# liuli33/CMLPL

Hardware: AMD Instinct MI355X
Metric: HSI patches/sec per training step (higher is better)
Workload: dtype f32 (convolutions: f32 operands as 3 exact bf16 pieces on the bf16 MFMA, 6 of 9 piece products, f32 accumulate, per-product worst case 2^-21 -- conv1's tap loops of the per-sample kernels as 2 fp16 pieces with power-of-two operand scales, 3 piece products, worst case 2^-20 / mean 2^-23, falling back; 1 GPU; B2: synthetic PaviaU-shaped patches 11x11x103, spectrum 103, 9 classes, 128 labelled + 128 unlabelled rows per GPU (batch 256), dual BaseNet2 fwd/bwd + contrastive/mutual losses + bank + Adam, epoch 1 (memory-bank smoothing active), in-kernel PCG4D noise / Philox dropout; global_batch=256, parallelism=dp1

## Files before the change

### cmlpl_amd/csrc/conv3x3.hip

```cpp
#include <stdlib.h>
#include <string.h>
#include <type_traits>

#ifndef CMLPL_ABL
#define CMLPL_ABL 0
#endif
#define CMLPL_UNR_F 1

#include "common.hpp"
#include "kernels.hpp"

namespace cmlpl {

constexpr int CS = 68;

__global__ void pack_weights_kernel(const float* __restrict__ params, long long pstride, PackInfo pi,
                                    float* __restrict__ packed) {
  const int net = blockIdx.y;
  const long long e = (long long)blockIdx.x * blockDim.x + threadIdx.x;
  if (e >= pi.stride) return;
  const float* P = params + (long long)net * pstride;
  float v;
  if (e < 4LL * PACK_B3) {
    const int which = (int)(e / PACK_B3);
// ... 85 lines not shown
#define STAMP(MODE_, i) do {} while (0)
#define STAMPG(MODE_, i) do {} while (0)
#endif

struct Conv3Args {
  const float* in; const uint8_t* mask_in; const float* wpk; const float* bias;
  float* out; uint8_t* mask_out;
  long long in_ns, mask_in_ns, wpk_ns, bias_ns, out_ns, mask_out_ns;
  int n, H, W, S;
  const float* w0t; const float* b0; float* a0out;
  long long w0t_ns, b0_ns;
  int C;
  float* xn_out;
  float* part0; long long part0_ns;
  int bp;
  XSrc xs;
  const float* w2f; long long w2f_ns;
  const float* b2; const float* wc; const float* bc; long long p_ns;
  const float* yin;
  const float* dropmask; float* dropgen; float* catd; float* ynorm; float* logits; float* feat;
  float* p2out; uint8_t* m2out;
  float dropout_p; int train, K;
  const float* dlogits; const float* dfeat; const float* hmask;
  const float* ynrm; const uint8_t* m2in; const float* w2d; long long w2d_ns;
  float* dy; float* dp2out; float* dp1out;
  const float* cube; int crows, ccols; long long pix0; long long* labels_out;
  uint32_t mg_hw, mg_w, mg_p2, mg_w2;
  const float* wpk16; long long wpk16_ns; const uint32_t* h2flag; long long h2flag_ns; int maxslot;
  int h2_noskip;
  int pairshift;
  int hkind;
  uint32_t* hstat;
  const long long* pix;
};

static inline uint32_t fdiv_magic(int d) { return d <= 1 ? 0u : (uint32_t)((0x100000000ULL + (uint32_t)d - 1) / (uint32_t)d); }
__device__ __forceinline__ int fdiv(int x, uint32_t mg) { return mg == 0u ? x : (int)__umulhi((uint32_t)x, mg); }
static inline void conv3_set_magics(Conv3Args& a) {
  const int H2 = a.H >> 1, W2 = a.W >> 1;
  a.mg_hw = fdiv_magic(a.H * a.W); a.mg_w = fdiv_magic(a.W); a.mg_p2 = fdiv_magic(H2 * W2); a.mg_w2 = fdiv_magic(W2);
}

__device__ __forceinline__ void wg_decode(const Conv3Args& a, int& net, int& s0) {
  net = (int)blockIdx.y; s0 = (int)blockIdx.x * a.S;
  if (a.pairshift != 0 && net == 1) { s0 += a.n >> 1; if (s0 >= a.n) s0 -= a.n; }
}
__device__ __forceinline__ int wg_infer_sample(const Conv3Args& a) {
  const int b = (int)blockIdx.x, per = (a.n + 7) >> 3;
  const int s = (b & 7) * per + (b >> 3);
  return ((b >> 3) < per && s < a.n) ? s : -1;
}

typedef float f32x4v __attribute__((ext_vector_type(4)));
__device__ __forceinline__ f32x4v mfma16(float a, float b, f32x4v c) {
  return __builtin_amdgcn_mfma_f32_16x16x4f32(a, b, c, 0, 0, 0);
}

constexpr int SLAB_MAXQ = 16;
constexpr int SLAB_RING = 7;
constexpr int SLAB_WIN = 4;
constexpr int SLAB_NUP = 7;
static_assert(SLAB_NUP == SLAB_RING, "the forward forms the noise of every chunk of a pass up front");
typedef __attribute__((address_space(3))) void slab_lds_void;
typedef __attribute__((address_space(1))) const void slab_gbl_void;
struct SlabRange { const float* xs; int nfl; };
__device__ __forceinline__ SlabRange slab_range(const XSrc& x, int net, int s, int per, int f4base, int nfl) {
// ... 977 lines not shown
    if (sample < a.n) {
      const float* p = c.img + (size_t)(s * c.IMG + (2 * ph + 1) * c.PW + 2 * pw + 1) * CS + c4 * 4;
      const float4 v00 = *(const float4*)p, v01 = *(const float4*)(p + CS);
      const float4 v10 = *(const float4*)(p + c.PW * CS), v11 = *(const float4*)(p + c.PW * CS + CS);
      const size_t g = ((size_t)sample * c.P2 + q) * 64 + c4 * 4;
      float4 o;
      o.x = (v00.x + v01.x + v10.x + v11.x) * 0.25f;
      o.y = (v00.y + v01.y + v10.y + v11.y) * 0.25f;
      o.z = (v00.z + v01.z + v10.z + v11.z) * 0.25f;
      o.w = (v00.w + v01.w + v10.w + v11.w) * 0.25f;
      if constexpr (STORE) *(float4*)(out + g) = o;
      if constexpr (STAT) pmx = mag_max4(pmx, o);
      if (img2 != nullptr) *(float4*)(img2 + (size_t)((ph + 1) * (c.W2 + 2) + pw + 1) * CS + c4 * 4) = o;
#define CMLPL_NIB(A, B, C, D) ((uint32_t)((relu_open(A) ? 1 : 0) | (relu_open(B) ? 2 : 0) | (relu_open(C) ? 4 : 0) | (relu_open(D) ? 8 : 0)))
      const uint32_t m = CMLPL_NIB(v00.x, v01.x, v10.x, v11.x) | (CMLPL_NIB(v00.y, v01.y, v10.y, v11.y) << 8) |
                         (CMLPL_NIB(v00.z, v01.z, v10.z, v11.z) << 16) | (CMLPL_NIB(v00.w, v01.w, v10.w, v11.w) << 24);
#undef CMLPL_NIB
      if constexpr (STORE) *(uint32_t*)(mo + g) = m;
    }
  }
  if constexpr (STAT) { if (statslot != nullptr) h2_publish_max(pmx, statslot); }
}

__device__ __forceinline__ long long logits_argmax(const float* v, int K) {
  int best = 0;
  float bv = v[0];
  for (int k = 1; k < K; ++k) {
    const float x = v[k];
    if (bv == bv && (x != x || x > bv)) { best = k; bv = x; }
  }
  return (long long)best;
}

template <int NW = 4, bool INFER = false>
__device__ __forceinline__ void conv3_fwd_tail(const Conv3Args& a, const Conv3Ctx& c, float* smem) {
  constexpr int NT = 64 * NW;
  const int tid = c.tid, lane = c.lane, wave = c.wave, net = c.net, sample = c.s0;
  const int PW2 = c.W2 + 2;
  const float* img2 = c.wbuf;
  float* row = smem;
  const int SF = 256, F = SF + FD, K = a.K;
  float* red = smem + F;
  const long long rs = (long long)net * a.n + sample;
  constexpr int PS2 = 36;
  const int NPX2 = (c.H2 + 2) * PW2, PLN = NPX2 * PS2;
  uint32_t* pl = (uint32_t*)(smem + 2048);
  auto split_planes = [&]() {
    for (int it = tid; it < NPX2 * 16; it += NT) {
      const int px = it >> 4, c4 = it & 15;
      const float4 v = *(const float4*)(img2 + (size_t)px * CS + 4 * c4);
      const float x[4] = {v.x, v.y, v.z, v.w};
      uint32_t u0[4], u1[4], u2[4];
#pragma unroll
      for (int q = 0; q < 4; ++q) {
        u0[q] = __float_as_uint(x[q]);
        const float r1 = x[q] - __uint_as_float(u0[q] & 0xffff0000u);
        u1[q] = __float_as_uint(r1);
        const float r2 = r1 - __uint_as_float(u1[q] & 0xffff0000u);
        u2[q] = __float_as_uint(r2);
      }
      uint32_t* d = pl + px * PS2 + 2 * c4;
      *(uint2*)(d) = make_uint2(hi_pair(u0[0], u0[1]), hi_pair(u0[2], u0[3]));
      *(uint2*)(d + PLN) = make_uint2(hi_pair(u1[0], u1[1]), hi_pair(u1[2], u1[3]));
      *(uint2*)(d + 2 * PLN) = make_uint2(hi_pair(u2[0], u2[1]), hi_pair(u2[2], u2[3]));
    }
  };
  static_assert(!(INFER && NW == 8), "inference from the cube: four-wave or eight-tile kernels");
  if (NW == 8 && wave >= 4) {
    __syncthreads();
    split_planes();
    __syncthreads();
    __syncthreads();
    __syncthreads();
    __syncthreads();
    return;
  }
  const int j = lane & 15, kg = lane >> 4;
  const uint4* wq = (const uint4*)(a.w2f + (long long)net * a.w2f_ns) + ((kg >> 1) * 6 + (wave >> 1)) * 64 + (kg & 1) * 32 +
                    16 * (wave & 1) + j;
  constexpr int C2_AHEAD = 3;
  uint4 bq[C2_AHEAD + 1][6];
#pragma unroll
  for (int t0 = 0; t0 < C2_AHEAD; ++t0)
#pragma unroll
    for (int ks = 0; ks < 2; ++ks)
#pragma unroll
      for (int pc = 0; pc < 3; ++pc) bq[t0][3 * ks + pc] = wq[((t0 * 4 + 2 * ks) * 3 + pc) * 128];
  const float4 y4 = *(const float4*)(a.yin + rs * FD + 4 * tid);
  const float bias2 = (a.b2 + (long long)net * a.p_ns)[wave * 16 + j];
  const float bcv = (a.bc + (long long)net * a.p_ns)[tid < K ? tid : 0];
  const float* wc = a.wc + (long long)net * a.p_ns;
  const int F4 = F >> 2, fb = wave * F4;
  float wv0[16][5];
#pragma unroll
  for (int q = 0; q < 16; ++q) {
    const float* wr = wc + (long long)(q < K ? q : K - 1) * F + fb + lane;
#pragma unroll
    for (int i = 0; i < 5; ++i) wv0[q][i] = wr[64 * i];
  }
  const int dmode = (!a.train || a.dropout_p <= 0.f) ? 0 : (a.dropmask != nullptr ? 1 : 2);
  const float keep_scale = 1.0f / (1.0f - a.dropout_p);
  float4 dm4[2];
#pragma unroll
  for (int q = 0; q < 2; ++q) {
    const int f0 = 1024 * q + 4 * tid;
    dm4[q] = make_float4(1.f, 1.f, 1.f, 1.f);
    if (f0 < F) {
      if (dmode == 1) {
        dm4[q] = *(const float4*)(a.dropmask + rs * F + f0);
      } else if (dmode == 2) {
        const unsigned long long gs = xsrc_global_sample(a.xs, sample);
        const float4 u = philox_uniform4(a.xs.seed, xsrc_step(a.xs), STREAM_DROPOUT + net, (gs * F + f0) >> 2);
        float4 m4;
        m4.x = (u.x >= a.dropout_p) ? keep_scale : 0.f; m4.y = (u.y >= a.dropout_p) ? keep_scale : 0.f;
        m4.z = (u.z >= a.dropout_p) ? keep_scale : 0.f; m4.w = (u.w >= a.dropout_p) ? keep_scale : 0.f;
        *(float4*)(a.dropgen + rs * F + f0) = m4;
        dm4[q] = m4;
      }
    }
  }
  if (CMLPL_ABL == 25) STAMP(0, 4);
  __syncthreads();
  if (CMLPL_ABL == 25) STAMP(0, 5);
  *(float4*)(row + SF + 4 * tid) = y4;
  split_planes();
  __syncthreads();
  if (CMLPL_ABL == 25) STAMP(0, 6);
  const uint32_t* ap0 = pl + (size_t)(((j >> 2) + 1) * PW2 + (j & 3) + 1) * PS2 + 4 * kg;
  f32x4v acc0 = {0.f, 0.f, 0.f, 0.f}, acc1 = {0.f, 0.f, 0.f, 0.f};
  auto mm = [](const uint4& x, const uint4& y, f32x4v cc) {
    return __builtin_amdgcn_mfma_f32_16x16x32_bf16(__builtin_bit_cast(bf16x8, x), __builtin_bit_cast(bf16x8, y), cc, 0, 0, 0);
  };
  uint4 af[2][6];
  auto read_a = [&](int tap, uint4 (&x)[6]) {
    const uint32_t* ap = ap0 + ((tap / 3 - 1) * PW2 + (tap % 3 - 1)) * PS2;
#pragma unroll
    for (int ks = 0; ks < 2; ++ks) {
      x[3 * ks] = *(const uint4*)(ap + 16 * ks); x[3 * ks + 1] = *(const uint4*)(ap + PLN + 16 * ks);
      x[3 * ks + 2] = *(const uint4*)(ap + 2 * PLN + 16 * ks);
    }
  };
  read_a(0, af[0]);
#pragma unroll
  for (int tap = 0; tap < 9; ++tap) {
    if (tap + C2_AHEAD < 9) {
#pragma unroll
      for (int ks = 0; ks < 2; ++ks)
#pragma unroll
        for (int pc = 0; pc < 3; ++pc)
          bq[(tap + C2_AHEAD) % (C2_AHEAD + 1)][3 * ks + pc] = wq[(((tap + C2_AHEAD) * 4 + 2 * ks) * 3 + pc) * 128];
    }
    if (tap + 1 < 9) read_a(tap + 1, af[(tap + 1) & 1]);
    const uint4 (&bcur)[6] = bq[tap % (C2_AHEAD + 1)];
    const uint4 (&acur)[6] = af[tap & 1];
#pragma unroll
    for (int ks = 0; ks < 2; ++ks) {
      const uint4 a1 = acur[3 * ks], a2 = acur[3 * ks + 1], a3 = acur[3 * ks + 2];
      const uint4 b1 = bcur[3 * ks], b2 = bcur[3 * ks + 1], b3 = bcur[3 * ks + 2];
      acc0 = mm(a1, b3, acc0); acc1 = mm(a2, b2, acc1); acc0 = mm(a3, b1, acc0);
      acc1 = mm(a1, b2, acc1); acc0 = mm(a2, b1, acc0); acc1 = mm(a1, b1, acc1);
    }
    __builtin_amdgcn_sched_group_barrier(0x020, 6, 0);
    __builtin_amdgcn_sched_group_barrier(0x100, 6, 0);
    __builtin_amdgcn_sched_group_barrier(0x008, 12, 0);
  }
  STAMP(0, 8);
  {
    const int co = wave * 16 + j;
    const float* res = img2 + (size_t)((kg + 1) * PW2 + 1) * CS + co;
    float r_[4];
#pragma unroll
    for (int r = 0; r < 4; ++r) r_[r] = relu_nan((acc0[r] + acc1[r]) + bias2 + res[r * CS]);
    const float s0 = r_[0] + r_[1], s1 = r_[2] + r_[3];
    const float t0 = s0 + __shfl_xor(s0, 16, 64), t1 = s1 + __shfl_xor(s1, 16, 64);
    const int dh = kg & 1;
    uint32_t n0 = (relu_open(r_[0]) ? 1u : 0u) | (relu_open(r_[1]) ? 2u : 0u);
    uint32_t n1 = (relu_open(r_[2]) ? 1u : 0u) | (relu_open(r_[3]) ? 2u : 0u);
    n0 <<= 2 * dh; n1 <<= 2 * dh;
    n0 |= (uint32_t)__shfl_xor((int)n0, 16, 64); n1 |= (uint32_t)__shfl_xor((int)n1, 16, 64);
    if (dh == 0) {
      const int ph = kg >> 1;
      const float o0 = t0 * 0.25f, o1 = t1 * 0.25f;
      if constexpr (!INFER) {
        float* p2 = a.p2out + (rs * 4 + ph * 2) * 64 + co;
        uint8_t* m2 = a.m2out + (rs * 4 + ph * 2) * 64 + co;
        p2[0] = o0; p2[64] = o1;
        m2[0] = (uint8_t)n0; m2[64] = (uint8_t)n1;
      }
      row[co * 4 + ph * 2] = o0;
      row[co * 4 + ph * 2 + 1] = o1;
    }
  }
  if (CMLPL_ABL == 25) STAMP(0, 12);
  float ss = (y4.x * y4.x + y4.y * y4.y) + (y4.z * y4.z + y4.w * y4.w);
  ss = wave_sum(ss);
  if (lane == 0) red[wave] = ss;
  __syncthreads();
  if (CMLPL_ABL == 25) STAMP(0, 13);
  if constexpr (!INFER) {
// ... 51 lines not shown
    }
    float t[16];
#pragma unroll
    for (int q = 0; q < 16; ++q) {
      float acc = 0.f;
#pragma unroll
      for (int i = 0; i < 5; ++i) acc = fmaf(xr[i], wv[q][i], acc);
      t[q] = acc;
    }
#pragma unroll
    for (int o = 32; o > 0; o >>= 1)
#pragma unroll
      for (int q = 0; q < 16; ++q) t[q] += __shfl_xor(t[q], o, 64);
    if (lane == 0) {
#pragma unroll
      for (int q = 0; q < 16; ++q)
        if (kc + q < K) part[wave * 64 + kc + q] = t[q];
    }
  }
  __syncthreads();
  if constexpr (INFER) {
    if (tid < K) {
      const float lg = ((part[tid] + part[64 + tid]) + (part[128 + tid] + part[192 + tid])) + bcv;
      part[256 + tid] = lg;
      if (a.logits != nullptr) a.logits[rs * K + tid] = lg;
    }
    __syncthreads();
    if (tid == 0) a.labels_out[rs] = logits_argmax(part + 256, K);
  } else {
    if (tid < K) a.logits[rs * K + tid] = ((part[tid] + part[64 + tid]) + (part[128 + tid] + part[192 + tid])) + bcv;
  }
}

template <int NW = 4>
__device__ __forceinline__ const float* conv3_bwd_head(const Conv3Args& a, float* smem, uint32_t (&mpre)[2]) {
  constexpr int NT = 64 * NW;
  const int tid = threadIdx.x, lane = tid & 63;
  const int wave = __builtin_amdgcn_readfirstlane(tid >> 6);
  int net, sample;
  wg_decode(a, net, sample);
  const int H2 = a.H >> 1, W2 = a.W >> 1, P2 = H2 * W2, PW2 = W2 + 2;
  const int SF = 256, F = SF + FD, K = a.K;
  float* img2 = smem + (size_t)(a.H + 2) * (a.W + 2) * CS;
  float* ext = img2 + WBUF + 128;
  float* dp1s = ext;
  float* dp2s = dp1s + P2 * 64;
  float* dls = dp2s + 256;
  float* red = dls + 64;
  const long long rs = (long long)net * a.n + sample;
#pragma unroll
  for (int q = 0; q < 2; ++q) {
    const int idx = tid + NT * q;
    mpre[q] = (idx < P2 * 16) ? *(const uint32_t*)(a.mask_in + (long long)net * a.mask_in_ns + ((size_t)sample * P2 + (idx >> 4)) * 64 + (idx & 15) * 4) : 0u;
  }
  if (NW == 8 && wave >= 4) {
    __syncthreads(); __syncthreads(); __syncthreads(); __syncthreads(); __syncthreads(); __syncthreads();
    return dp1s;
  }
  const int l31 = lane & 31, hh = lane >> 5;
  const int nt = wave & 1, kh2 = wave >> 1;
  const uint4* wq = (const uint4*)(a.w2d + (long long)net * a.w2d_ns) + lane;
  constexpr int C2_AHEAD = 3;
  uint4 bq[C2_AHEAD + 1][6];
#pragma unroll
  for (int t0 = 0; t0 < C2_AHEAD; ++t0)
#pragma unroll
    for (int q = 0; q < 2; ++q)
#pragma unroll
      for (int pc = 0; pc < 3; ++pc) bq[t0][3 * q + pc] = wq[(size_t)t0 * TAPW + (((kh2 * 2 + q) * 3 + pc) * 2 + nt) * 64];
  if (tid < 64) dls[tid] = (tid < K) ? a.dlogits[rs * K + tid] : 0.f;
  const float* y = a.yin + rs * FD;
  const float* df = (a.dfeat != nullptr) ? a.dfeat + rs * FD : nullptr;
  const float norm = a.ynrm[rs];
  float yv[4], dv[4];
#pragma unroll
  for (int q = 0; q < 4; ++q) {
    yv[q] = y[tid + 256 * q];
    dv[q] = (df != nullptr) ? df[tid + 256 * q] : 0.f;
  }
  const uint32_t m2pre = (tid < 64) ? *(const uint32_t*)(a.m2in + (rs * 4 + (tid >> 4)) * 64 + (tid & 15) * 4) : 0u;
  const float* wc = a.wc + (long long)net * a.p_ns;
  const float* dm = (a.hmask != nullptr) ? a.hmask + rs * F : nullptr;
  float dmv[5];
#pragma unroll
  for (int it = 0; it < 5; ++it) dmv[it] = (dm != nullptr) ? dm[tid + 256 * it] : 1.f;
  float wv0[16][5];
#pragma unroll
  for (int q = 0; q < 16; ++q) {
    const float* wr = wc + (long long)(q < K ? q : K - 1) * F + tid;
#pragma unroll
    for (int it = 0; it < 5; ++it) wv0[q][it] = wr[256 * it];
  }
  {
    const float4 z4 = make_float4(0.f, 0.f, 0.f, 0.f);
    for (int i = tid; i < 1024; i += 256) ((float4*)img2)[i] = z4;
    const int PW = a.W + 2, IMG = (a.H + 2) * PW;
    for (int i = tid; i < IMG * (CS / 4); i += 256) ((float4*)smem)[i] = z4;
    int* lut = (int*)(img2 + WBUF);
    const int HWl = a.H * a.W;
    for (int m = tid; m < 128; m += 256) {
      const int mm = (m < HWl) ? m : 0;
      const int r = mm / a.W, cc = mm - r * a.W;
// ... 54 lines not shown
    const float4 d = *(const float4*)(dp2s + pp * 64 + c4 * 4);
    const uint32_t m = m2pre;
    uint32_t zmx = 0u;
#pragma unroll
    for (int sub = 0; sub < 4; ++sub) {
      float4 v;
      v.x = ((m >> sub) & 1u) ? d.x * 0.25f : 0.f;
      v.y = ((m >> (8 + sub)) & 1u) ? d.y * 0.25f : 0.f;
      v.z = ((m >> (16 + sub)) & 1u) ? d.z * 0.25f : 0.f;
      v.w = ((m >> (24 + sub)) & 1u) ? d.w * 0.25f : 0.f;
      const int h = 2 * ph + (sub >> 1), w = 2 * pw + (sub & 1);
      *(float4*)(img2 + (size_t)((h + 1) * PW2 + w + 1) * CS + c4 * 4) = v;
      zmx = mag_max4(zmx, v);
    }
    if (a.hstat != nullptr) {
      zmx = wave_mag_max(zmx);
      if (tid == 0) { a.hstat[(3 * 2 + net) * a.n + sample] = zmx; ((uint32_t*)smem)[a.maxslot + 1] = zmx; }
    }
  }
  __syncthreads();
  const bool z2skip = a.hstat != nullptr && a.h2_noskip == 0 && ((const volatile uint32_t*)smem)[a.maxslot + 1] == 0u &&
                      a.h2flag[(long long)net * a.h2flag_ns] == 0u;
  STAMP(1, 5);
  const int mg2 = (65536 + W2 - 1) / W2;
  const int phA = (l31 * mg2) >> 16;
  const int posA = l31 < P2 ? (phA + 1) * PW2 + (l31 - phA * W2) + 1 : 0;
  const float* ap = img2 + (size_t)posA * CS + kh2 * 32 + hh * 8;
  f32x16 acc = zero16();
  auto raw_ptr = [&](int u) {
    const int tap = u >> 1;
    const int toff = ((tap / 3 - 1) * PW2 + (tap % 3 - 1)) * CS;
    return ((l31 < P2) ? ap + toff : ap) + 16 * (u & 1);
  };
  ASplit cur;
  float4 rn0, rn1;
  if (!z2skip) {
  {
    const float* p0 = raw_ptr(0);
    a_split(*(const float4*)p0, *(const float4*)(p0 + 4), cur.p1, cur.p2, cur.p3);
    const float* p1 = raw_ptr(1);
    rn0 = *(const float4*)p1; rn1 = *(const float4*)(p1 + 4);
  }
#pragma unroll
  for (int u = 0; u < 18; ++u) {
    const int tap = u >> 1, q = u & 1;
    if (q == 0 && tap + C2_AHEAD < 9) {
#pragma unroll
      for (int q2 = 0; q2 < 2; ++q2)
#pragma unroll
        for (int pc = 0; pc < 3; ++pc)
          bq[(tap + C2_AHEAD) % (C2_AHEAD + 1)][3 * q2 + pc] =
              wq[(size_t)(tap + C2_AHEAD) * TAPW + (((kh2 * 2 + q2) * 3 + pc) * 2 + nt) * 64];
    }
    if (q == 0) __builtin_amdgcn_sched_barrier(0);
    float4 rnn0 = rn0, rnn1 = rn1;
    if (u + 2 < 18) {
      const float* p2 = raw_ptr(u + 2);
      rnn0 = *(const float4*)p2; rnn1 = *(const float4*)(p2 + 4);
    }
    const uint4 (&bcur)[6] = bq[tap % (C2_AHEAD + 1)];
    acc = mfma_b3(cur.p1, cur.p2, cur.p3, bcur[3 * q], bcur[3 * q + 1], bcur[3 * q + 2], acc);
    ASplit nxt = cur;
    if (u + 1 < 18) a_split(rn0, rn1, nxt.p1, nxt.p2, nxt.p3);
    if (u + 2 < 18) __builtin_amdgcn_sched_group_barrier(0x100, 2, 0);
    SchedInterleave<6>::run();
    cur = nxt; rn0 = rnn0; rn1 = rnn1;
  }
  }
  STAMP(1, 6);
// ... 437 lines not shown
        if (p < P2) {
          const float v = (acc[r] + xch[r * 64 + lane]) + res[r];
          dp1s[p * 64 + ci] = v;
          dp1g[p * 64 + ci] = v;
        }
      }
    }
  }
  __syncthreads();
  STAMP(1, 11);
  return dp1s;
}

template <int MODE, int MTW, int TAIL = 0, int NW = 4, int TPW = 8 / NW, bool KSG = false, bool H2X = false>
__global__ __launch_bounds__(64 * NW, ((MODE >= 2 || KSG) && NW == 4 ? 2 : 1)) void conv3x3_kernel(Conv3Args a) {
  static_assert(!KSG || (MODE < 2 && MTW == 1 && TAIL == 0 && NW == 4 && TPW == 2), "KSG: four waves, S = 1, four tiles");
  static_assert(!H2X || (MODE >= 2 && TAIL == 1 && (NW == 8 || TPW == 2)) || (MODE < 2 && TAIL == 0 && (KSG || NW == 8)),
                "H2X: the per-sample kernels with tail / head; the general kernels with one sample per workgroup");
  extern __shared__ __attribute__((aligned(16))) float smem[];
  if constexpr (H2X) { if (threadIdx.x == 0) { smem[a.maxslot] = 0.f; smem[a.maxslot + 1] = 0.f; } }
  constexpr int NT = 64 * NW;
  constexpr int KMT = NW * TPW / 2;
  constexpr int LUTN = (MODE >= 2) ? KMT * 32 : MTW * NW * 32;
  constexpr bool BIG = (KMT == 8);
  constexpr bool INFER = (MODE == 2 && TAIL >= 2);
  if constexpr (INFER) { if (wg_infer_sample(a) < 0) return; }
  if (CMLPL_ABL == 26) return;
  Conv3Ctx c;
  STAMPG(MODE & 1, 0);
  const float* dp_lds = nullptr;
  uint32_t mpre[2] = {0u, 0u};
  if constexpr (MODE == 3 && TAIL) {
    if constexpr (BIG) dp_lds = conv3_bwd_head_g(a, smem, mpre);
    else dp_lds = conv3_bwd_head<NW>(a, smem, mpre);
  }
  conv3_stage<MODE, NW, TPW, INFER ? (TAIL & 1) + 1 : 0, H2X, (INFER && TAIL >= 4)>(a, smem, LUTN, c, dp_lds, mpre);
  STAMPG(MODE & 1, 1);
  const int tid = c.tid, lane = c.lane, l31 = c.l31, hh = c.hh, wave = c.wave, net = c.net, s0 = c.s0;
  const int HW = c.HW, PW = c.PW, S = c.S, PX = c.PX, npx = c.npx;
  float* img = c.img; float* wbuf = c.wbuf; int* lut = c.lut; const float4* wg = c.wg;
  const TapRegs wp = c.wp;
  const int MT = (npx + 31) >> 5;
  int abase[MTW];
  f32x16 acc[MTW][2];
  constexpr bool KS = (MODE >= 2) || KSG;
  const int RL = MT - NW * (MTW - 1);
  const bool nsplit = !KS && NW == 8 && MTW >= 2 && (RL == 1 || RL == 5);
  int last_tile = wave + NW * (MTW - 1), nmask = 3;
  if (nsplit && wave == RL - 1) nmask = 1;
  else if (nsplit && wave == RL) { last_tile = MT - 1; nmask = 2; }
  auto slot_tile = [&](int t) { return t == MTW - 1 ? last_tile : wave + NW * t; };
  if constexpr (!KS) {
#pragma unroll
    for (int t = 0; t < MTW; ++t) {
      abase[t] = lut[slot_tile(t) * 32 + l31] * CS + 8 * hh;
      acc[t][0] = zero16();
      acc[t][1] = zero16();
    }
  }
  int ab2[TPW];
  f32x16 acc2[TPW][2];
  if (KS) {
#pragma unroll
    for (int t = 0; t < TPW; ++t) {
      ab2[t] = lut[(TPW * (wave >> 1) + t) * 32 + l31] * CS + 8 * hh;
      acc2[t][0] = zero16();
      acc2[t][1] = zero16();
// ... 118 lines not shown
      const int nm = (t == MTW - 1) ? nmask : 3;
      if (tile < MT) {
        int pos[16];
        float x0[16], x1[16];
#pragma unroll
        for (int r = 0; r < 16; ++r) {
          const int m = tile * 32 + acc_row(r, lane);
          pos[r] = lut[m < npx ? m : 0] * CS;
        }
#pragma unroll
        for (int r = 0; r < 16; ++r) { x0[r] = img[pos[r] + l31]; x1[r] = img[pos[r] + 32 + l31]; }
#pragma unroll
        for (int r = 0; r < 16; ++r) {
          const int m = tile * 32 + acc_row(r, lane);
          if (m < npx) {
            if (nm & 1) img[pos[r] + l31] = relu_nan(acc[t][0][r] + bv0 + x0[r]);
            if (nm & 2) img[pos[r] + 32 + l31] = relu_nan(acc[t][1][r] + bv1 + x1[r]);
          }
        }
      }
    }
    }
    if (TAIL) {
      const float4 z4 = make_float4(0.f, 0.f, 0.f, 0.f);
      for (int i = tid; i < (BIG ? WBUF / 4 : 1024); i += NT) ((float4*)wbuf)[i] = z4;
    }
    STAMP(0, 10);
    __syncthreads();
    STAMP(0, 11);
    conv3_pool_store<NT, !INFER, H2X>(a, c, TAIL ? wbuf : nullptr, (H2X && a.hstat != nullptr) ? smem + a.maxslot + 1 : nullptr);
    STAMP(0, 7);
    if constexpr (TAIL != 0) {
      if constexpr (BIG) conv3_fwd_tail_g<INFER>(a, c, smem);
      else conv3_fwd_tail<NW, INFER>(a, c, smem);
    }
    if constexpr (H2X) {
      if (a.hstat != nullptr && tid == 0) a.hstat[(1 * 2 + net) * a.n + s0] = ((const volatile uint32_t*)smem)[a.maxslot + 1];
    }
  } else if (MODE == 3) {
    const int C = a.C, BP = a.bp;
    float vv[TPW][16];
    {
      int pos[16];
#pragma unroll
      for (int r = 0; r < 16; ++r) {
        const int m = ot * 32 + acc_row(r, lane);
        pos[r] = lut[m < PX ? m : 0] * CS + 32 * nt0 + l31;
      }
#pragma unroll
      for (int r = 0; r < 16; ++r)
#pragma unroll
        for (int i = 0; i < TPW; ++i) vv[i][r] = img[pos[r] + 32 * i];
#pragma unroll
      for (int r = 0; r < 16; ++r)
#pragma unroll
        for (int i = 0; i < TPW; ++i) vv[i][r] += own[i][r];
    }
    __syncthreads();
    float* slab = smem;
    float* dal = smem + (C < BP ? C : BP) * HW;
    const int Cw = conv0_partial_rows(C);
    float* pp = a.part0 + (long long)net * a.part0_ns + (size_t)s0 * ((size_t)Cw * 64 + 64);
    bool zskip = false;
    if constexpr (H2X) {
      if (a.hstat != nullptr) zskip = hzero && a.h2_noskip == 0 && (a.hstat[(0 * 2 + net) * a.n + s0] >> 23) < 255u;
    }
    SlabRange rg = slab_range(a.xs, net, s0, C * HW, 0, (C < BP ? C : BP) * HW);
// ... 439 lines not shown
  *v = Conv3Variant{};
  if (H != W || K < 1 || K > 64 || C < 1) return false;
  BigGeom g;
  if (conv3_big_geom(H, W, &g) && conv3_big_fwd_lds(g, C) <= LDS_MAX) {
    *v = per_sample(8, 2, conv3_big_fwd_lds(g, C));
    return true;
  }
  if (switches().fuse_conv0 == 0 || switches().fuse_tail == 0 || H * W > 128 || H < 8 || W < 8) return false;
  if (H2 / 2 != 2 || W2 / 2 != 2 || (H2 + 2) * (W2 + 2) * CS > 4096 || !conv3_divide_exact(W, 128)) return false;
  const size_t lds = conv3_fused_lds(H, W, C, conv3_lds(1, H, W, 1));
  if (2 * lds > LDS_MAX) return false;
  *v = per_sample(4, 2, lds);
  return true;
}

static Conv3Args conv3_args(int mode, int n, int H, int W, int S, const float* in, const uint8_t* mask_in, float* out,
                            uint8_t* mask_out) {
  Conv3Args a{};
  const long long window = (long long)n * H * W * 64, pooled = (long long)n * (H / 2) * (W / 2) * 64;
  a.in = in; a.mask_in = mask_in; a.out = out; a.mask_out = mask_out;
  if (in) a.in_ns = mode == 0 ? window : pooled;
  if (mask_in) a.mask_in_ns = pooled;
  if (out) a.out_ns = mode == 1 ? window : pooled;
  if (mask_out) a.mask_out_ns = pooled;
  a.n = n; a.H = H; a.W = W; a.S = S;
  conv3_set_magics(a);
  a.h2_noskip = switches().f16x2 == 4 || switches().zero_skip == 0;
  return a;
}
static void conv3_args_h2x(Conv3Args& a, const Conv3Variant& v, const float* wpk16, long long wpk16_ns, const uint32_t* h2flag,
                           uint32_t* hstat) {
  a.wpk16 = wpk16; a.wpk16_ns = wpk16_ns; a.h2flag = h2flag; a.h2flag_ns = wpk16_ns; a.hstat = hstat; a.maxslot = v.maxslot;
}

template <int MODE, int MTW, int TAIL, int NW, int TPW, bool KSG, bool H2X>
static hipError_t launch_conv3_k(const Conv3Args& a, dim3 grid, size_t lds, hipStream_t st) {
  static DevOnce attr_once;
  if (lds > LDS_MAX) return hipErrorInvalidValue;
  hipError_t e = ensure_max_lds(attr_once, conv3x3_kernel<MODE, MTW, TAIL, NW, TPW, KSG, H2X>);
  if (e != hipSuccess) return e;
  hipLaunchKernelGGL((conv3x3_kernel<MODE, MTW, TAIL, NW, TPW, KSG, H2X>), grid, dim3(64 * NW), lds, st, a);
  return hipGetLastError();
}
template <int MODE>
static hipError_t launch_conv3_small(const Conv3Args& a, dim3 grid, size_t lds, hipStream_t st) {
  static DevOnce attr_once;
  hipError_t e = ensure_max_lds(attr_once, conv3x3_small_kernel<MODE>);
  if (e != hipSuccess) return e;
  hipLaunchKernelGGL((conv3x3_small_kernel<MODE>), grid, dim3(256), lds, st, a);
  return hipGetLastError();
}

struct Conv3Kernel {
  int mode, mtw, tail, nw, tpw; bool ks, h2x;
  hipError_t (*launch)(const Conv3Args&, dim3, size_t, hipStream_t);
};
#define CMLPL_K(...) {__VA_ARGS__, launch_conv3_k<__VA_ARGS__>}
static const Conv3Kernel conv3_kernels[] = {
    CMLPL_K(0, 1, 0, 4, 2, true, true),
    CMLPL_K(1, 1, 0, 4, 2, true, true),
    CMLPL_K(0, 1, 0, 8, 1, false, true),
    CMLPL_K(1, 1, 0, 8, 1, false, true),
    CMLPL_K(0, 2, 0, 8, 1, false, true),
    CMLPL_K(1, 2, 0, 8, 1, false, true),
    CMLPL_K(0, 1, 0, 4, 2, true, false),
    CMLPL_K(1, 1, 0, 4, 2, true, false),
// ... 42 lines not shown
      return k.launch(a, grid, v.lds, st);
  return hipErrorInvalidValue;
}

hipError_t launch_conv3(const Conv3Variant& v, int mode, int nets, int n, int H, int W, const float* in, const uint8_t* mask_in,
                        const float* wpk, long long wpk_ns, const float* bias, long long bias_ns,
                        float* out, uint8_t* mask_out, hipStream_t st, const Conv3H2& h2) {
  if (v.S < 1) return hipErrorInvalidValue;
  Conv3Args a = conv3_args(mode, n, H, W, v.S, in, mask_in, out, mask_out);
  a.wpk = wpk; a.wpk_ns = wpk_ns; a.bias = bias; a.bias_ns = bias_ns;
  if (v.h2x) { conv3_args_h2x(a, v, h2.wpk16, h2.wpk16_ns, h2.h2flag, h2.hstat); a.hkind = h2.kind; }
  const dim3 grid((n + v.S - 1) / v.S, nets);
  return launch_conv3_variant(mode, 0, v, a, grid, st);
}

hipError_t launch_conv3_fused(const NetRoute& r, int nets, int n, int C, int H, int W, const XSrc& xs, const float* w0t,
                              long long w0t_ns, const float* b0, long long b0_ns, float* a0out, const float* wpk,
                              long long wpk_ns, const float* bias, long long bias_ns, float* out, uint8_t* mask_out,
                              const FwdTail* tail, hipStream_t st, float* xn_out) {
  const Conv3Variant& v = r.fwd_ps;
  if (r.fwd != (tail != nullptr ? ROUTE_A : ROUTE_B)) return hipErrorInvalidValue;
  Conv3Args a = conv3_args(2, n, H, W, 1, nullptr, nullptr, out, mask_out);
  a.wpk = wpk; a.wpk_ns = wpk_ns; a.bias = bias; a.bias_ns = bias_ns;
  a.w0t = w0t; a.w0t_ns = w0t_ns; a.b0 = b0; a.b0_ns = b0_ns; a.a0out = a0out; a.C = C; a.xn_out = xn_out;
  a.xs = xs;
  if (tail == nullptr) return launch_conv3_variant(2, 0, v, a, dim3(n, nets), st);
  a.w2f = tail->w2f; a.w2f_ns = tail->w2f_ns; a.b2 = tail->b2; a.wc = tail->wc; a.bc = tail->bc; a.p_ns = tail->p_ns;
  a.yin = tail->y; a.dropmask = tail->dropmask; a.dropgen = tail->dropgen; a.catd = tail->catd; a.ynorm = tail->ynorm;
  a.logits = tail->logits; a.feat = tail->feat; a.p2out = tail->p2; a.m2out = tail->m2;
  a.dropout_p = tail->dropout_p; a.train = tail->train; a.K = tail->K;
  if (v.h2x) {
    if (tail->w1h == nullptr || tail->h2flag == nullptr) return hipErrorInvalidValue;
    conv3_args_h2x(a, v, tail->w1h, tail->w1h_ns, tail->h2flag, tail->hstat);
  }
  return launch_conv3_variant(2, 1, v, a, dim3(n, nets), st);
}

hipError_t launch_conv3_infer(const Conv3Variant& v, int n, int C, int H, int W, const float* cube, int crows, int ccols,
                              long long pix0, const float* w0t, const float* b0, const float* wpk, const float* bias,
                              const FwdTail& t, long long* labels_out, hipStream_t st, const InferNets* nn, const ViewKey* view) {
  const int nets = nn != nullptr ? nn->nets : 1;
  if (v.S != 1 || n < 1 || !cube || !labels_out || nets < 1 || nets > 2) return hipErrorInvalidValue;
  if ((long long)crows * ccols * C >= (1LL << 31) || W / 2 > crows || W / 2 > ccols) return hipErrorInvalidValue;
  Conv3Args a = conv3_args(2, n, H, W, 1, nullptr, nullptr, nullptr, nullptr);
  a.wpk = wpk; a.bias = bias;
  a.w0t = w0t; a.b0 = b0; a.C = C;
  a.w2f = t.w2f; a.b2 = t.b2; a.wc = t.wc; a.bc = t.bc; a.yin = t.y; a.logits = t.logits; a.K = t.K;
  a.cube = cube; a.crows = crows; a.ccols = ccols; a.pix0 = pix0; a.labels_out = labels_out;
  if (nn != nullptr) {
    a.wpk_ns = nn->packed_ns; a.w0t_ns = nn->packed_ns; a.w2f_ns = nn->packed_ns;
    a.bias_ns = nn->param_ns; a.b0_ns = nn->param_ns; a.p_ns = nn->param_ns;
    a.pix = nn->pix;
  }
  const dim3 grid(8 * ((n + 7) / 8), nets);
  if (view != nullptr && view->sigma != 0.f) {
    a.xs.sigma = view->sigma; a.xs.seed = view->seed; a.xs.step = view->view;
    return launch_conv3_variant(2, a.pix != nullptr ? 5 : 4, v, a, grid, st);
  }
  return launch_conv3_variant(2, a.pix != nullptr ? 3 : 2, v, a, grid, st);
}

hipError_t launch_conv3_fused_bwd(const NetRoute& r, int nets, int n, int C, int H, int W, const float* dpool,
                                  const uint8_t* mask, const float* wpk, long long wpk_ns, const XSrc& xs, float* part0,
                                  long long part0_ns, const BwdHead* head, hipStream_t st) {
  const Conv3Variant& v = r.bwd_ps;
  if (r.bwd != (head != nullptr ? ROUTE_A : ROUTE_B)) return hipErrorInvalidValue;
  if (xs.sigma != 0.f || xs.sel.lab_idx != nullptr || xs.sel.unl_idx != nullptr) return hipErrorInvalidValue;
  Conv3Args a = conv3_args(3, n, H, W, 1, dpool, mask, nullptr, nullptr);
  a.wpk = wpk; a.wpk_ns = wpk_ns;
  a.C = C; a.xs = xs; a.part0 = part0; a.part0_ns = part0_ns; a.bp = v.bp;
  if (head == nullptr) return launch_conv3_variant(3, 0, v, a, dim3(n, nets), st);
  a.dlogits = head->dlogits; a.dfeat = head->dfeat; a.hmask = head->mask; a.wc = head->wc; a.p_ns = head->p_ns;
  a.yin = head->y; a.ynrm = head->ynorm; a.m2in = head->m2; a.w2d = head->w2d; a.w2d_ns = head->w2d_ns;
  a.dy = head->dy; a.dp2out = head->dp2; a.dp1out = head->dp1; a.K = head->K;
  a.pairshift = (nets == 2 && switches().bwd_pair != 0) ? 1 : 0;
  if (v.h2x) {
    if (head->w1h == nullptr || head->h2flag == nullptr) return hipErrorInvalidValue;
    conv3_args_h2x(a, v, head->w1h, head->w1h_ns, head->h2flag, head->hstat);
  }
  return launch_conv3_variant(3, 1, v, a, dim3(n, nets), st);
}

}
```

### cmlpl_amd/csrc/kernels.hpp

```cpp
#pragma once
#include <hip/hip_runtime.h>
#include <stdint.h>
#include <stddef.h>
#include <stdlib.h>
#include <atomic>

#include "common.hpp"

namespace cmlpl {

constexpr int PACK_CONV = 9 * 64 * 64;
constexpr int PACK_B3 = PACK_CONV * 3 / 2;
constexpr int PACK_PER_NET = 4 * PACK_B3 + PACK_CONV;
__host__ __device__ inline long long pack_off_b3(int , int , int which) { return (long long)which * PACK_B3; }
__host__ __device__ inline long long pack_off_frag() { return 4LL * PACK_B3; }
__host__ __device__ inline int conv_b3_index(int tap, int k, int n, int p) {
  return ((((tap * 4 + (k >> 4)) * 3 + p) * 2 + (n >> 5)) * 64 + ((k >> 3) & 1) * 32 + (n & 31)) * 8 + (k & 7);
}
__host__ __device__ inline long long pack_off_w0t() { return PACK_PER_NET; }
__host__ __device__ inline long long pack_off_wst(int C) { return PACK_PER_NET + (long long)((C + 1) & ~1) * 64; }
__host__ __device__ inline long long pack_off_w0b3(int C, int bands) { return pack_off_wst(C) + (long long)bands * 1024; }
__host__ __device__ inline long long pack_off_w0b3_end(int C, int bands) { return pack_off_w0b3(C, bands) + (long long)((C + 15) / 16) * 1536; }
constexpr int H2_WEXP = 13;
constexpr int PACK_H2 = PACK_CONV;
// ... 133 lines not shown
hipError_t launch_feat_norm(int nets, int n, const float* y, float* ynorm, float* feat, long long feat_ns, hipStream_t st);
struct GemmTN {
  const float* A; const float* B; float* C; float* bias;
  const float* bias_in; long long bias_in_bstride; int relu;
  long long a_bstride, b_bstride, c_bstride, bias_bstride;
  int lda, ldb, ldc, M, N, R, batches;
  float scale;
  int b_seg_rows = 0; long long b_seg_stride = 0;
};
hipError_t launch_gemm_tn(const GemmTN& g, hipStream_t st);
hipError_t launch_gemm_tn2(const GemmTN& g0, const GemmTN& g1, hipStream_t st);

hipError_t launch_head_fwd(int nets, int n, int HW4, int K, const float* p2, const float* y, const float* dropmask,
                           float* dropgen, float dropout_p, int train, uint64_t seed, uint64_t step,
                           int nlab, int lab0, int unl_base,
                           const float* wc, const float* bc, long long pstride,
                           float* catd, float* ynorm, float* logits, float* feat, hipStream_t st,
                           DynRef dyn = DynRef());
hipError_t launch_head_bwd(int nets, int n, int HW4, int K, const float* dlogits, const float* dfeat,
                           const float* dropmask, const float* wc, long long pstride,
                           const float* y, const float* ynorm,
                           float* dy, float* dp2, hipStream_t st);
hipError_t launch_dy_fixup(int nets, int n, const float* y, const float* ynorm, const float* dfeat, float* dy,
                           hipStream_t st);

struct Switches {
  int fuse_conv0, fuse_conv0_bwd, fuse_tail, fuse_spe;
  int fuse_big;
  int conv3_nw8;
  int conv0a;
  int zero_skip;
  int bwd_pair;
  int f16x2;
  int conv3_ks;
  int ks8;
  int conv3_s, conv0_dma, conv0_ps;
  int wgrad3_u, wgrad3_cspl, wgrad3_r, wgrad3_ru, wgrad3_rg, wgrad3_pg1, wgrad3_pg2, wgrad3_b3, wgrad3_pair;
  int pair_wide, pair_nbw, pair_mb, pair16, pair_tall;
  int dfeat_lds;
  int mb_fast, unsup_onewg, unsup_3l, ntx_mfma;
  int ntx_ncw;
};
inline Switches read_switches() {
    auto env = [](const char* name, int dflt) { const char* v = getenv(name); return v ? atoi(v) : dflt; };
    Switches w;
    w.fuse_conv0 = env("CMLPL_FUSE_CONV0", 1); w.fuse_conv0_bwd = env("CMLPL_FUSE_CONV0_BWD", 1);
    w.fuse_tail = env("CMLPL_FUSE_TAIL", 1); w.fuse_spe = env("CMLPL_FUSE_SPE", 1);
    w.ks8 = env("CMLPL_KS8", -1); w.fuse_big = env("CMLPL_FUSE_BIG", 1); w.conv3_nw8 = env("CMLPL_CONV3_NW8", 1); w.conv3_ks = env("CMLPL_CONV3_KS", 1); w.conv0a = env("CMLPL_CONV0A", 1); w.f16x2 = env("CMLPL_F16X2", 1); w.bwd_pair = env("CMLPL_BWD_PAIR", 1); w.zero_skip = env("CMLPL_ZERO_SKIP", 1);
    w.conv3_s = env("CMLPL_CONV3_S", 0); w.conv0_dma = env("CMLPL_CONV0_DMA", 1); w.conv0_ps = env("CMLPL_CONV0_PS", 0);
    w.wgrad3_u = env("CMLPL_WGRAD3_U", 0); w.wgrad3_cspl = env("CMLPL_WGRAD3_CSPL", 0); w.wgrad3_r = env("CMLPL_WGRAD3_R", 1);
    w.wgrad3_ru = env("CMLPL_WGRAD3_RU", 0); w.wgrad3_rg = env("CMLPL_WGRAD3_RG", 0);
    w.wgrad3_pg1 = env("CMLPL_WGRAD3_PG1", 0); w.wgrad3_pg2 = env("CMLPL_WGRAD3_PG2", 0);
    w.wgrad3_b3 = env("CMLPL_WGRAD3_B3", 1); w.wgrad3_pair = env("CMLPL_WGRAD3_PAIR", 1);
    w.pair_wide = env("CMLPL_PAIR_WIDE", -1); w.pair_nbw = env("CMLPL_PAIR_NBW", 0); w.pair_mb = env("CMLPL_PAIR_MB", 0);
    w.pair16 = env("CMLPL_PAIR16", 1); w.pair_tall = env("CMLPL_PAIR_TALL", -1);
    w.dfeat_lds = env("CMLPL_DFEAT_LDS", -1);
    w.mb_fast = env("CMLPL_MB_FAST", 1); w.unsup_onewg = env("CMLPL_UNSUP_ONEWG", 1); w.unsup_3l = env("CMLPL_UNSUP_3L", 1);
    w.ntx_mfma = env("CMLPL_NTX_MFMA", 1); w.ntx_ncw = env("CMLPL_NTX_NCW", 0);
    return w;
}
inline Switches& switches_table() {
  static Switches sw = read_switches();
  return sw;
}
inline const Switches& switches() { return switches_table(); }

inline int device_cus() {
  static std::atomic<int> cache[64];
  int dev = 0;
  if (hipGetDevice(&dev) != hipSuccess) return 256;
  int v = cache[dev & 63].load(std::memory_order_relaxed);
  if (v == 0) {
    hipDeviceProp_t prop;
    v = (hipGetDeviceProperties(&prop, dev) == hipSuccess && prop.multiProcessorCount > 0) ? prop.multiProcessorCount : 256;
    cache[dev & 63].store(v, std::memory_order_relaxed);
  }
  return v;
}

struct LossArgs {
  const float* logits; const float* feat; const int64_t* labels;
// ... 97 lines not shown
```

Baseline: 1.761 million patches/s.

## Run conv2 fwd tail and bwd head on fp16 two-piece MFMA path

```diff
diff --git a/cmlpl_amd/csrc/conv3x3.hip b/cmlpl_amd/csrc/conv3x3.hip
--- a/cmlpl_amd/csrc/conv3x3.hip
+++ b/cmlpl_amd/csrc/conv3x3.hip
@@ -141,6 +141,7 @@
   int hkind;
   uint32_t* hstat;
   const long long* pix;
+  int h2c2;
 };
 
 static inline uint32_t fdiv_magic(int d) { return d <= 1 ? 0u : (uint32_t)((0x100000000ULL + (uint32_t)d - 1) / (uint32_t)d); }
@@ -1184,7 +1185,7 @@
   return (long long)best;
 }
 
-template <int NW = 4, bool INFER = false>
+template <int NW = 4, bool INFER = false, bool H2X = false>
 __device__ __forceinline__ void conv3_fwd_tail(const Conv3Args& a, const Conv3Ctx& c, float* smem) {
   constexpr int NT = 64 * NW;
   const int tid = c.tid, lane = c.lane, wave = c.wave, net = c.net, sample = c.s0;
@@ -1217,10 +1218,38 @@
       *(uint2*)(d + 2 * PLN) = make_uint2(hi_pair(u2[0], u2[1]), hi_pair(u2[2], u2[3]));
     }
   };
+  bool spec = false, c2h = false;
+  float c2sc = 1.f, c2inv = 1.f;
+  if constexpr (H2X) spec = a.h2c2 != 0 && a.hstat != nullptr && a.h2flag[(long long)net * a.h2flag_ns] == 0u;
+  auto split_planes_h = [&](float sc) {
+    for (int it = tid; it < NPX2 * 16; it += NT) {
+      const int px = it >> 4, c4 = it & 15;
+      const float4 v = *(const float4*)(img2 + (size_t)px * CS + 4 * c4);
+      const float x0 = v.x * sc, x1 = v.y * sc, x2 = v.z * sc, x3 = v.w * sc;
+      const f16x2v p0 = __builtin_bit_cast(f16x2v, __builtin_amdgcn_cvt_pkrtz(x0, x1));
+      const f16x2v p1 = __builtin_bit_cast(f16x2v, __builtin_amdgcn_cvt_pkrtz(x2, x3));
+      uint32_t* d = pl + px * PS2 + 2 * c4;
+      *(uint2*)(d) = make_uint2(__builtin_bit_cast(uint32_t, p0), __builtin_bit_cast(uint32_t, p1));
+      *(uint2*)(d + PLN) = make_uint2(__builtin_bit_cast(uint32_t, __builtin_amdgcn_cvt_pkrtz(x0 - (float)p0[0], x1 - (float)p0[1])),
+                                      __builtin_bit_cast(uint32_t, __builtin_amdgcn_cvt_pkrtz(x2 - (float)p1[0], x3 - (float)p1[1])));
+    }
+  };
+  auto c2_decide = [&]() {
+    if constexpr (H2X) {
+      if (spec) {
+        const uint32_t mxb = __builtin_amdgcn_readfirstlane(((const volatile uint32_t*)smem)[a.maxslot + 1]);
+        const uint32_t e = mxb >> 23;
+        c2h = (e >= 40u && e <= 200u) || mxb == 0u;
+        c2sc = mxb == 0u ? 1.f : __uint_as_float((268u - e) << 23);
+        c2inv = mxb == 0u ? 1.f : __uint_as_float((e - 27u - (uint32_t)(H2_WEXP - 13)) << 23);
+      }
+    }
+  };
   static_assert(!(INFER && NW == 8), "inference from the cube: four-wave or eight-tile kernels");
   if (NW == 8 && wave >= 4) {
     __syncthreads();
-    split_planes();
+    c2_decide();
+    if (c2h) split_planes_h(c2sc); else split_planes();
     __syncthreads();
     __syncthreads();
     __syncthreads();
@@ -1232,24 +1261,42 @@
                     16 * (wave & 1) + j;
   constexpr int C2_AHEAD = 3;
   uint4 bq[C2_AHEAD + 1][6];
-#pragma unroll
-  for (int t0 = 0; t0 < C2_AHEAD; ++t0)
-#pragma unroll
-    for (int ks = 0; ks < 2; ++ks)
-#pragma unroll
-      for (int pc = 0; pc < 3; ++pc) bq[t0][3 * ks + pc] = wq[((t0 * 4 + 2 * ks) * 3 + pc) * 128];
+  auto b3_fill = [&]() {
+#pragma unroll
+    for (int t0 = 0; t0 < C2_AHEAD; ++t0)
+#pragma unroll
+      for (int ks = 0; ks < 2; ++ks)
+#pragma unroll
+        for (int pc = 0; pc < 3; ++pc) bq[t0][3 * ks + pc] = wq[((t0 * 4 + 2 * ks) * 3 + pc) * 128];
+  };
+  const uint4* wqh = nullptr;
+  constexpr int H_AHEAD = C2_AHEAD;
+  auto hq = [&](int tap, int i) -> uint4& { return bq[tap % (H_AHEAD + 1)][i]; };
+  if constexpr (H2X) {
+    wqh = (const uint4*)(a.wpk16 + (long long)net * a.wpk16_ns + 2LL * PACK_H2) + ((kg >> 1) * 4 + (wave >> 1)) * 64 +
+          (kg & 1) * 32 + 16 * (wave & 1) + j;
+    if (spec) {
+#pragma unroll
+      for (int t0 = 0; t0 < H_AHEAD; ++t0)
+#pragma unroll
+        for (int i = 0; i < 4; ++i) hq(t0, i) = wqh[(t0 * 8 + 4 * (i >> 1) + (i & 1)) * 128];
+    }
+  }
+  if (!spec) b3_fill();
   const float4 y4 = *(const float4*)(a.yin + rs * FD + 4 * tid);
   const float bias2 = (a.b2 + (long long)net * a.p_ns)[wave * 16 + j];
   const float bcv = (a.bc + (long long)net * a.p_ns)[tid < K ? tid : 0];
   const float* wc = a.wc + (long long)net * a.p_ns;
   const int F4 = F >> 2, fb = wave * F4;
+  constexpr int WV_EARLY = H2X ? 4 : 16;
   float wv0[16][5];
-#pragma unroll
-  for (int q = 0; q < 16; ++q) {
+  auto wv_load = [&](int q) {
     const float* wr = wc + (long long)(q < K ? q : K - 1) * F + fb + lane;
 #pragma unroll
     for (int i = 0; i < 5; ++i) wv0[q][i] = wr[64 * i];
-  }
+  };
+#pragma unroll
+  for (int q = 0; q < WV_EARLY; ++q) wv_load(q);
   const int dmode = (!a.train || a.dropout_p <= 0.f) ? 0 : (a.dropmask != nullptr ? 1 : 2);
   const float keep_scale = 1.0f / (1.0f - a.dropout_p);
   float4 dm4[2];
@@ -1275,7 +1322,9 @@
   __syncthreads();
   if (CMLPL_ABL == 25) STAMP(0, 5);
   *(float4*)(row + SF + 4 * tid) = y4;
-  split_planes();
+  c2_decide();
+  if (c2h) split_planes_h(c2sc); else split_planes();
+  if (spec && !c2h) b3_fill();
   __syncthreads();
   if (CMLPL_ABL == 25) STAMP(0, 6);
   const uint32_t* ap0 = pl + (size_t)(((j >> 2) + 1) * PW2 + (j & 3) + 1) * PS2 + 4 * kg;
@@ -1292,6 +1341,35 @@
       x[3 * ks + 2] = *(const uint4*)(ap + 2 * PLN + 16 * ks);
     }
   };
+  if (c2h) {
+    auto mh = [](const uint4& x, const uint4& y, f32x4v cc) {
+      return __builtin_amdgcn_mfma_f32_16x16x32_f16(__builtin_bit_cast(f16x8v, x), __builtin_bit_cast(f16x8v, y), cc, 0, 0, 0);
+    };
+    uint4 ah[2][4];
+    auto read_h = [&](int tap, uint4 (&x)[4]) {
+      const uint32_t* ap = ap0 + ((tap / 3 - 1) * PW2 + (tap % 3 - 1)) * PS2;
+#pragma unroll
+      for (int ks = 0; ks < 2; ++ks) { x[2 * ks] = *(const uint4*)(ap + 16 * ks); x[2 * ks + 1] = *(const uint4*)(ap + PLN + 16 * ks); }
+    };
+    read_h(0, ah[0]);
+#pragma unroll
+    for (int tap = 0; tap < 9; ++tap) {
+      const uint4 g[4] = {hq(tap, 0), hq(tap, 1), hq(tap, 2), hq(tap, 3)};
+      if (tap + H_AHEAD < 9) {
+#pragma unroll
+        for (int i = 0; i < 4; ++i) hq(tap + H_AHEAD, i) = wqh[((tap + H_AHEAD) * 8 + 4 * (i >> 1) + (i & 1)) * 128];
+      }
+      if (tap + 1 < 9) read_h(tap + 1, ah[(tap + 1) & 1]);
+      const uint4 (&h)[4] = ah[tap & 1];
+      acc0 = mh(h[1], g[0], acc0); acc1 = mh(h[0], g[1], acc1); acc0 = mh(h[0], g[0], acc0);
+      acc1 = mh(h[3], g[2], acc1); acc0 = mh(h[2], g[3], acc0); acc1 = mh(h[2], g[2], acc1);
+      __builtin_amdgcn_sched_group_barrier(0x020, 4, 0);
+      __builtin_amdgcn_sched_group_barrier(0x100, 4, 0);
+      __builtin_amdgcn_sched_group_barrier(0x008, 6, 0);
+    }
+#pragma unroll
+    for (int r = 0; r < 4; ++r) { acc0[r] = (acc0[r] + acc1[r]) * c2inv; acc1[r] = 0.f; }
+  } else {
   read_a(0, af[0]);
 #pragma unroll
   for (int tap = 0; tap < 9; ++tap) {
@@ -1316,7 +1394,10 @@
     __builtin_amdgcn_sched_group_barrier(0x100, 6, 0);
     __builtin_amdgcn_sched_group_barrier(0x008, 12, 0);
   }
+  }
   STAMP(0, 8);
+#pragma unroll
+  for (int q = WV_EARLY; q < 16; ++q) wv_load(q);
   {
     const int co = wave * 16 + j;
     const float* res = img2 + (size_t)((kg + 1) * PW2 + 1) * CS + co;
@@ -1434,7 +1515,7 @@
   }
 }
 
-template <int NW = 4>
+template <int NW = 4, bool H2X = false>
 __device__ __forceinline__ const float* conv3_bwd_head(const Conv3Args& a, float* smem, uint32_t (&mpre)[2]) {
   constexpr int NT = 64 * NW;
   const int tid = threadIdx.x, lane = tid & 63;
@@ -1464,12 +1545,29 @@
   const uint4* wq = (const uint4*)(a.w2d + (long long)net * a.w2d_ns) + lane;
   constexpr int C2_AHEAD = 3;
   uint4 bq[C2_AHEAD + 1][6];
+  auto b3_fill = [&]() {
 #pragma unroll
   for (int t0 = 0; t0 < C2_AHEAD; ++t0)
 #pragma unroll
     for (int q = 0; q < 2; ++q)
 #pragma unroll
       for (int pc = 0; pc < 3; ++pc) bq[t0][3 * q + pc] = wq[(size_t)t0 * TAPW + (((kh2 * 2 + q) * 3 + pc) * 2 + nt) * 64];
+  };
+  bool spec = false;
+  const uint4* wqh = nullptr;
+  constexpr int H_AHEAD = 5;
+  auto hq = [&](int tap, int i) -> uint4& { const int sl = (tap % (H_AHEAD + 1)) * 4 + i; return bq[sl / 6][sl % 6]; };
+  if constexpr (H2X) {
+    spec = a.h2c2 != 0 && a.hstat != nullptr && a.h2flag[(long long)net * a.h2flag_ns] == 0u;
+    wqh = (const uint4*)(a.wpk16 + (long long)net * a.wpk16_ns + 2LL * PACK_H2) + lane;
+    if (spec) {
+#pragma unroll
+      for (int t0 = 0; t0 < H_AHEAD; ++t0)
+#pragma unroll
+        for (int i = 0; i < 4; ++i) hq(t0, i) = wqh[(size_t)t0 * TAPH + (((kh2 * 2 + (i >> 1)) * 2 + (i & 1)) * 2 + nt) * 64];
+    }
+  }
+  if (!spec) b3_fill();
   if (tid < 64) dls[tid] = (tid < K) ? a.dlogits[rs * K + tid] : 0.f;
   const float* y = a.yin + rs * FD;
   const float* df = (a.dfeat != nullptr) ? a.dfeat + rs * FD : nullptr;
@@ -1590,9 +1688,53 @@
     const int toff = ((tap / 3 - 1) * PW2 + (tap % 3 - 1)) * CS;
     return ((l31 < P2) ? ap + toff : ap) + 16 * (u & 1);
   };
+  bool c2h = false;
+  float c2sc = 1.f, c2inv = 1.f;
+  if constexpr (H2X) {
+    if (spec) {
+      const uint32_t mxb = __builtin_amdgcn_readfirstlane(((const volatile uint32_t*)smem)[a.maxslot + 1]);
+      const uint32_t e = mxb >> 23;
+      c2h = (e >= 40u && e <= 200u) || mxb == 0u;
+      c2sc = mxb == 0u ? 1.f : __uint_as_float((268u - e) << 23);
+      c2inv = mxb == 0u ? 1.f : __uint_as_float((e - 27u - (uint32_t)(H2_WEXP - 13)) << 23);
+    }
+  }
+  if (!z2skip && c2h) {
+    HSplit hc;
+    float4 rn0, rn1;
+    {
+      const float* p0 = raw_ptr(0);
+      h_split(*(const float4*)p0, *(const float4*)(p0 + 4), c2sc, hc.p1, hc.p2);
+      const float* p1 = raw_ptr(1);
+      rn0 = *(const float4*)p1; rn1 = *(const float4*)(p1 + 4);
+    }
+#pragma unroll
+    for (int u = 0; u < 18; ++u) {
+      const int tap = u >> 1, q = u & 1;
+      if (q == 0 && tap + H_AHEAD < 9) {
+#pragma unroll
+        for (int i = 0; i < 4; ++i)
+          hq(tap + H_AHEAD, i) = wqh[(size_t)(tap + H_AHEAD) * TAPH + (((kh2 * 2 + (i >> 1)) * 2 + (i & 1)) * 2 + nt) * 64];
+      }
+      if (q == 0) __builtin_amdgcn_sched_barrier(0);
+      float4 rnn0 = rn0, rnn1 = rn1;
+      if (u + 2 < 18) {
+        const float* p2 = raw_ptr(u + 2);
+        rnn0 = *(const float4*)p2; rnn1 = *(const float4*)(p2 + 4);
+      }
+      acc = mfma_h2(hc.p1, hc.p2, hq(tap, 2 * q), hq(tap, 2 * q + 1), acc);
+      HSplit nxt = hc;
+      if (u + 1 < 18) h_split(rn0, rn1, c2sc, nxt.p1, nxt.p2);
+      if (u + 2 < 18) __builtin_amdgcn_sched_group_barrier(0x100, 2, 0);
+      SchedInterleave<3>::run();
+      hc = nxt; rn0 = rnn0; rn1 = rnn1;
+    }
+#pragma unroll
+    for (int r = 0; r < 16; ++r) acc[r] *= c2inv;
+  } else if (!z2skip) {
   ASplit cur;
   float4 rn0, rn1;
-  if (!z2skip) {
+  if (spec) b3_fill();
   {
     const float* p0 = raw_ptr(0);
     a_split(*(const float4*)p0, *(const float4*)(p0 + 4), cur.p1, cur.p2, cur.p3);
@@ -2096,7 +2238,7 @@
   uint32_t mpre[2] = {0u, 0u};
   if constexpr (MODE == 3 && TAIL) {
     if constexpr (BIG) dp_lds = conv3_bwd_head_g(a, smem, mpre);
-    else dp_lds = conv3_bwd_head<NW>(a, smem, mpre);
+    else dp_lds = conv3_bwd_head<NW, H2X>(a, smem, mpre);
   }
   conv3_stage<MODE, NW, TPW, INFER ? (TAIL & 1) + 1 : 0, H2X, (INFER && TAIL >= 4)>(a, smem, LUTN, c, dp_lds, mpre);
   STAMPG(MODE & 1, 1);
@@ -2281,7 +2423,7 @@
     STAMP(0, 7);
     if constexpr (TAIL != 0) {
       if constexpr (BIG) conv3_fwd_tail_g<INFER>(a, c, smem);
-      else conv3_fwd_tail<NW, INFER>(a, c, smem);
+      else conv3_fwd_tail<NW, INFER, H2X>(a, c, smem);
     }
     if constexpr (H2X) {
       if (a.hstat != nullptr && tid == 0) a.hstat[(1 * 2 + net) * a.n + s0] = ((const volatile uint32_t*)smem)[a.maxslot + 1];
@@ -2787,6 +2929,7 @@
                            uint32_t* hstat) {
   a.wpk16 = wpk16; a.wpk16_ns = wpk16_ns; a.h2flag = h2flag; a.h2flag_ns = wpk16_ns; a.hstat = hstat; a.maxslot = v.maxslot;
 }
+static int conv3_h2c2(const Conv3Variant& v) { return (v.h2x && !v.big && switches().h2_conv2 != 0) ? 1 : 0; }
 
 template <int MODE, int MTW, int TAIL, int NW, int TPW, bool KSG, bool H2X>
 static hipError_t launch_conv3_k(const Conv3Args& a, dim3 grid, size_t lds, hipStream_t st) {
@@ -2895,6 +3038,7 @@
   if (v.h2x) {
     if (tail->w1h == nullptr || tail->h2flag == nullptr) return hipErrorInvalidValue;
     conv3_args_h2x(a, v, tail->w1h, tail->w1h_ns, tail->h2flag, tail->hstat);
+    a.h2c2 = conv3_h2c2(v);
   }
   return launch_conv3_variant(2, 1, v, a, dim3(n, nets), st);
 }
@@ -2940,6 +3084,7 @@
   if (v.h2x) {
     if (head->w1h == nullptr || head->h2flag == nullptr) return hipErrorInvalidValue;
     conv3_args_h2x(a, v, head->w1h, head->w1h_ns, head->h2flag, head->hstat);
+    a.h2c2 = conv3_h2c2(v);
   }
   return launch_conv3_variant(3, 1, v, a, dim3(n, nets), st);
 }
diff --git a/cmlpl_amd/csrc/kernels.hpp b/cmlpl_amd/csrc/kernels.hpp
--- a/cmlpl_amd/csrc/kernels.hpp
+++ b/cmlpl_amd/csrc/kernels.hpp
@@ -189,6 +189,7 @@
   int zero_skip;
   int bwd_pair;
   int f16x2;
+  int h2_conv2;
   int conv3_ks;
   int ks8;
   int conv3_s, conv0_dma, conv0_ps;
@@ -204,6 +205,7 @@
     w.fuse_conv0 = env("CMLPL_FUSE_CONV0", 1); w.fuse_conv0_bwd = env("CMLPL_FUSE_CONV0_BWD", 1);
     w.fuse_tail = env("CMLPL_FUSE_TAIL", 1); w.fuse_spe = env("CMLPL_FUSE_SPE", 1);
     w.ks8 = env("CMLPL_KS8", -1); w.fuse_big = env("CMLPL_FUSE_BIG", 1); w.conv3_nw8 = env("CMLPL_CONV3_NW8", 1); w.conv3_ks = env("CMLPL_CONV3_KS", 1); w.conv0a = env("CMLPL_CONV0A", 1); w.f16x2 = env("CMLPL_F16X2", 1); w.bwd_pair = env("CMLPL_BWD_PAIR", 1); w.zero_skip = env("CMLPL_ZERO_SKIP", 1);
+    w.h2_conv2 = env("CMLPL_H2_CONV2", 1);
     w.conv3_s = env("CMLPL_CONV3_S", 0); w.conv0_dma = env("CMLPL_CONV0_DMA", 1); w.conv0_ps = env("CMLPL_CONV0_PS", 0);
     w.wgrad3_u = env("CMLPL_WGRAD3_U", 0); w.wgrad3_cspl = env("CMLPL_WGRAD3_CSPL", 0); w.wgrad3_r = env("CMLPL_WGRAD3_R", 1);
     w.wgrad3_ru = env("CMLPL_WGRAD3_RU", 0); w.wgrad3_rg = env("CMLPL_WGRAD3_RG", 0);
```

Measured after the change: 1.772 million patches/s (median of 6 runs). No clear change (+0.6%).
